# lilinitsy/skele-raytracer

Measured on AMD Instinct MI355X. Metric: Mrays/sec + frame ms, 1920x1080 gillum=16 spheres2.scn, higher is better.
Workload: dtype f32

## Files before the change

skele_raytracer_amd/csrc/launch.h:

```cpp
#pragma once

#include <hip/hip_runtime.h>
#include <stddef.h>
#include <stdint.h>

#include "render_params.h"

enum { SKR_LEVEL0_RUN = 0, SKR_LEVEL0_BUILD, SKR_LEVEL0_REPLAY };
enum { SKR_PIX_NONE = 0, SKR_PIX_NODE, SKR_PIX_BACKGROUND, SKR_PIX_TRIANGLE };

constexpr int SKR_NODE_LEVELS_MAX = 33;
struct NodePlan {
	bool flat = false;
	int levels = 0;
	uint32_t band_nblk = 0;
	uint64_t nodes_max[SKR_NODE_LEVELS_MAX] = {};
	uint32_t cap[SKR_NODE_LEVELS_MAX] = {};
	size_t off_nodes[SKR_NODE_LEVELS_MAX] = {}, off_shade[SKR_NODE_LEVELS_MAX] = {}, off_recs[SKR_NODE_LEVELS_MAX] = {}, off_res[SKR_NODE_LEVELS_MAX] = {}, off_ixh[SKR_NODE_LEVELS_MAX] = {};
	size_t off_ctr = 0, ctr_bytes = 0, total = 0, banded = 0;
	size_t off_cls = 0, off_sums = 0;
	size_t off_girow = 0;
	int level0 = SKR_LEVEL0_RUN;
	size_t lds_leaf = 0;
	size_t lds = 0;
};

constexpr int SKR_GLEVELS_MAX = 64;
struct GPlan {
	int levels = 0;
	uint32_t band_rows = 0;
	uint64_t nodes_max[SKR_GLEVELS_MAX + 1] = {};
	uint32_t cap[SKR_GLEVELS_MAX + 1] = {};
	size_t off_nodes[SKR_GLEVELS_MAX + 1] = {}, off_recs[SKR_GLEVELS_MAX + 1] = {}, off_res[SKR_GLEVELS_MAX + 1] = {}, off_hdr[SKR_GLEVELS_MAX + 1] = {};
	size_t off_ctr = 0, ctr_bytes = 0, total = 0;
};

struct QueryTrees {
	const float4 *tree;
	const float4 *trace;
	uint32_t stride;
	int32_t nchunks;
	int32_t cones, trace_cones;
	float4 ball;
};

struct ShadeRays {
	const float4 *rays;
	const uint32_t *keys;
	float *out;
	uint32_t n, ray0;
	QueryTrees trees;
};
constexpr uint32_t SKR_SHADE_ROW = 1024;

struct TriShadows {
	QueryTrees trees;
};

struct GenericFeatures {
	bool tri_shadows = false;
	bool sphere_tree = false;
	bool spot = false;
	bool soft = false;
	TriShadows shadows{};
	SphereTree stree{};
	SpotLights spots{};
	SoftLights softs{};
};

enum SkrPath { SKR_PATH_DIRECT = 0, SKR_PATH_NODES, SKR_PATH_GENERIC };

struct LaunchPlan {
	SkrPath path = SKR_PATH_DIRECT;
	const char *variant = "direct_v3";
	size_t scratch_bytes = 0;
	size_t acc_bytes = 0;
	size_t lds_bytes = 0;
	size_t off_ctr = 0;
	int levels = 0;
	NodePlan nodes;
	GPlan generic;
	GenericFeatures features;
};

static inline size_t skr_scene_lds_bytes(const RenderParams &p) { return ((size_t) 4 * p.n_spheres + 1 + 2 * p.n_lights) * 16; }

constexpr size_t SKR_PREFIX_LDS = ((size_t) SKR_PREFIX_WORDS * sizeof(uint32_t) + 15) & ~(size_t) 15;
static inline size_t skr_scene_kernels_lds(const RenderParams &p) { return skr_scene_lds_bytes(p) + 32 + SKR_PREFIX_LDS; }
static inline size_t skr_lights_lds_bytes(const RenderParams &p) { return ((size_t) 1 + 2 * p.n_lights) * 16; }
static inline size_t skr_lights_kernels_lds(const RenderParams &p) { return skr_lights_lds_bytes(p) + 32 + SKR_PREFIX_LDS; }

static inline uint32_t skr_tree_arity(const RenderParams &p) { return (uint32_t) (p.monte_carlo ? p.num_path_traces : 0) + (p.legacy_reflect ? 2u * (uint32_t) p.n_lights : 0u); }

struct ScratchLayout {
	size_t off = 0;
	size_t take(size_t bytes) { const size_t o = off; off += (bytes + 255) & ~(size_t) 255; return o; }
};

template <class Fits>
static uint32_t skr_largest_band(uint32_t all, Fits fits)
{
	if(fits(all)) return all;
	uint32_t lo = 1, hi = all;
	if(!fits(lo)) return 0;
	while(hi - lo > 1)
	{
		const uint32_t mid = lo + (hi - lo) / 2;
		if(fits(mid)) lo = mid;
		else hi = mid;
	}
	return lo;
}

enum SkrLeafShape { SKR_LEAF_RUNTIME = 0, SKR_LEAF_POINT1 = 1, SKR_LEAF_POINT2 = 2 };
static inline SkrLeafShape skr_leaf_shape(const RenderParams &p)
{
	if(!(p.sw.shadow_mask & SKR_SW_LEAF_SHAPE)) return SKR_LEAF_RUNTIME;
	if(p.n_tris != 0 || p.gi_index == nullptr || p.gi_wide != 0) return SKR_LEAF_RUNTIME;
	if(!p.use_shadows || p.shadow_masks == nullptr) return SKR_LEAF_RUNTIME;
	if(p.pow_steps > 7) return SKR_LEAF_RUNTIME;
	return p.n_lights == 2 ? SKR_LEAF_POINT2 : p.n_lights == 1 ? SKR_LEAF_POINT1 : SKR_LEAF_RUNTIME;
}

bool skr_plan_launch(const RenderParams &p, size_t lds_limit, LaunchPlan &lp, const GenericFeatures &f);
const char *skr_features_conflict(const GenericFeatures &f, bool legacy_reflect, bool shade_triangles, bool fog);
const char *skr_generic_variant(bool query, const GenericFeatures &f);
hipError_t skr_launch_render(const RenderParams &p, const LaunchPlan &lp, hipStream_t stream, const SkrTimingHook *hook);
hipError_t skr_launch_debug(int op, const void *d_in, void *d_out, uint32_t n, hipStream_t stream);
bool skr_nodes_plan(const RenderParams &p, size_t lds_limit, NodePlan &pl);
hipError_t skr_launch_nodes(const RenderParams &p, const NodePlan &pl, hipStream_t stream, const SkrTimingHook *hook);
hipError_t skr_nodes_level_count(const void *scratch, size_t off_ctr, int level, uint32_t *n);
bool skr_generic_plan(const RenderParams &p, GPlan &pl, bool sphere_tree = false);
hipError_t skr_launch_generic(const RenderParams &p, const GPlan &pl, hipStream_t stream, const SkrTimingHook *hook, const GenericFeatures &f, const ShadeRays *q = nullptr);
struct PrimaryKey {
	int32_t width, height;
	uint32_t tile_rows, first_tile, tile_stride, out_rows;
	const uint32_t *tile_table;
	uint64_t tile_table_id;
	float inv_width, inv_height, aspect, angle;
	f3 cam_pos, cam_dir, cam_up, cam_right, background;
	int32_t n_spheres, n_tris, n_lights;
	const float4 *scene, *cam_ec, *tri_chunks;
	int32_t tri_chunk_size, tri_cones, n_tri_chunks;
	int32_t use_shadows, pow_steps, num_path_traces, max_depth, flat, levels;
	const void *gi_index, *gi_surface;
	uint32_t band_nblk;
	const void *scratch;
	const void *counters;
	size_t off_ctr, off_nodes0, off_shade0, off_cls, off_sums, off_girow, total;
};
bool skr_primary_key(const RenderParams &p, const NodePlan &pl, uint64_t tile_table_id, PrimaryKey &key);
hipError_t skr_launch_wave(const RenderParams &p, size_t lds, hipStream_t stream);
hipError_t skr_launch_primary(const RenderParams &p, dim3 grid, size_t lds, hipStream_t stream);
hipError_t skr_launch_primary_build(const RenderParams &p, dim3 grid, size_t lds, uint8_t *cls, unsigned long long *sums, hipStream_t stream);
hipError_t skr_launch_primary_replay(const RenderParams &p, const uint8_t *cls, const unsigned long long *sums, hipStream_t stream);
hipError_t skr_launch_resolve(const RenderParams &p, hipStream_t stream);
hipError_t skr_launch_camec(const float4 *geom, int ns, f3 cam_pos, float4 *out, hipStream_t stream);
struct TraceScene {
	const float4 *geom;
	const float4 *tris;
	QueryTrees trees;
	int32_t ns, nt, chunk;
	f3 cam;
};
hipError_t skr_launch_trace(const TraceScene &s, const float4 *rays, uint32_t n, bool any_hit, void *out, hipStream_t stream, const SphereTree *st = nullptr);
hipError_t skr_launch_camera_rays(const RenderParams &p, float4 *rays, hipStream_t stream);
struct DenoiseScratch {
	float4 *img[2];
	float4 *guide;
	uint32_t *cls;
};
hipError_t skr_launch_denoise(const DenoiseScratch &b, uint32_t w, uint32_t h, const float *rgbf, const float4 *hits, const float *var, int iterations,
							  float *out_rgbf, uint8_t *out_rgb, hipStream_t stream);
hipError_t skr_launch_accumulate(float *acc, const float *frame, size_t n, int first, hipStream_t stream);
hipError_t skr_launch_resolve_accumulated(const float *acc, uint32_t passes, uint32_t width, uint32_t out_rows, uint32_t height, uint32_t tile_rows,
										  uint32_t first_tile, uint32_t tile_stride, const uint32_t *tile_table, uint8_t *rgb, float *rgbf, hipStream_t stream);
struct AdaptiveScratch {
	float4 *st;
	uint2 *st2;
	uint32_t *list[2];
	uint32_t *blocks;
	uint32_t *count;
	float4 *rays;
	float *shade;
	float *sacc;
};
struct AdaptiveRule {
	uint32_t min_passes, max_passes;
	float threshold;
};
constexpr float SKR_ADAPTIVE_CROSSOVER = 0.5f;
size_t skr_adaptive_scratch_bytes(uint64_t pixels);
AdaptiveScratch skr_adaptive_carve(void *base, uint64_t pixels);
hipError_t skr_launch_adaptive_fold(const AdaptiveScratch &s, const float *frame, const uint32_t *list, uint32_t m, int first, hipStream_t stream);
hipError_t skr_launch_adaptive_select(const AdaptiveScratch &s, const AdaptiveRule &rule, const uint32_t *in, uint32_t m, uint32_t *out, hipStream_t stream);
hipError_t skr_launch_adaptive_rays(const RenderParams &p, const uint32_t *list, uint32_t m, float4 *rays, hipStream_t stream);
hipError_t skr_launch_adaptive_sample(const AdaptiveScratch &s, const uint32_t *list, uint32_t m, uint32_t sample, uint32_t samples, hipStream_t stream);
hipError_t skr_launch_adaptive_resolve(const AdaptiveScratch &s, uint64_t pixels, uint8_t *rgb, float *rgbf, uint32_t *passes, float *var, hipStream_t stream);
```

skele_raytracer_amd/csrc/render_nodes.hip:

```cpp
#include <hip/hip_runtime.h>
#include <stdint.h>
#include <stdlib.h>
#include <string.h>

#include <vector>

#include "launch.h"
#include "wave_common.h"

namespace {

constexpr uint32_t PC_HIT0 = 1u, PC_HIT1 = 2u, PC_BLACK0 = 4u, PC_BLACK1 = 8u;
constexpr int IXH_ROWS = 3;
constexpr int NQ_CAP = 176;
constexpr int NQ_PRE = NQ_CAP - 128;
constexpr int NQ_F = 5;
constexpr int NWIN = 4;
constexpr int WIN_FLOATS = 2 * 3 * 64;
constexpr int LEAF2_WAVE_FLOATS = NQ_CAP * NQ_F + NWIN * WIN_FLOATS;

typedef const RenderParams __attribute__((address_space(4))) *LaunchArgs;
SKR_DEV const RenderParams &launch_args()
{
	LaunchArgs k = (LaunchArgs) __builtin_amdgcn_kernarg_segment_ptr();
	asm volatile("" : "+s"(k));
	return *(const RenderParams *) k;
}

SKR_DEV bool classify_child(const SceneView &sv, f3 co, f3 d, float two_a, float four_a, const BestState &s, bool &black)
{
	black = false;
	if(sv.nt > 0)
	{
		const float tmin = (s.best >= 0) ? near_root(two_a, s.b, s.D) : __builtin_inff();
		black = any_triangle_closer(sv, RayConst{co, d, two_a, four_a}, tmin);
	}
	return !black && s.best >= 0;
}

}

#ifndef SKR_TRACE_LOOP
#define SKR_TRACE_LOOP 1
#endif
#if SKR_TRACE_LOOP
#define SKR_TRACE_STRIDE gridDim.x
#else
#define SKR_TRACE_STRIDE 0x40000000u
#undef SKR_TRACE_GRID_MAX
#define SKR_TRACE_GRID_MAX 0x7fffffffu
#endif
#ifndef SKR_TRACE_WAVES
#define SKR_TRACE_WAVES 0
#endif
#if SKR_TRACE_WAVES
#define SKR_TRACE_ATTR __attribute__((amdgpu_waves_per_eu(SKR_TRACE_WAVES, SKR_TRACE_WAVES)))
#else
#define SKR_TRACE_ATTR
#endif
template <bool TRIS, bool GIM>
__global__ __launch_bounds__(256) SKR_TRACE_ATTR void skr_trace_kernel(const RenderParams)
{
	extern __shared__ __align__(16) unsigned char lds_raw[];
	float4 *lds4 = reinterpret_cast<float4 *>(lds_raw);
	const RenderParams &p = launch_args();
	const uint32_t N = (uint32_t) p.num_path_traces, PP = (N + 1u) >> 1;
	const uint64_t n_pairs = (uint64_t) *p.nd_count * PP;
	if((uint64_t) blockIdx.x * 256u >= n_pairs) return;
	stage_scene(p, lds4, TRIS);
	const int tid = threadIdx.x, lane = tid & 63;
	Counters cn{0, 0, 0};
	for(uint32_t blk = blockIdx.x; (uint64_t) blk * 256u < n_pairs; blk += SKR_TRACE_STRIDE)
	{
	const RenderParams &p = launch_args();
	const SceneView sv = scene_view(p, lds4, TRIS);
	const uint32_t chunk = blk * 4u + (uint32_t) (tid >> 6);
	const uint64_t tp = (uint64_t) chunk * 64u + (uint32_t) lane;
	const bool valid = tp < n_pairs;
	const uint32_t node = valid ? (uint32_t) (tp / PP) : 0u, j = valid ? (uint32_t) (tp - (uint64_t) node * PP) : 0u;
	const bool second = valid && 2u * j + 1u < N;
	bool hit0 = false, hit1 = false;
	float4 rec0 = make_float4(0, 0, 0, 0), rec1 = rec0;
	bool black0 = false, black1 = false;
	if(valid)
	{
		const float4 *row = p.nd_src + (size_t) node * 2;
		const float4 a0 = row[0], a1 = row[1];
		const f3 co = mk3(a0.x, a0.y, a0.z), Nn = mk3(a0.w, a1.x, a1.y);
		const uint32_t pixel = __float_as_uint(a1.z), node_id = __float_as_uint(a1.w);
		f3 nt, nb;
		tangent_basis(Nn, nt, nb);
		uint32_t rnd[4];
		philox4x32(pixel, p.aa_index, node_id, j, p.seed_lo, p.seed_hi, rnd);
		const float q1a = u31_to_unit(rnd[0]), q2a = u31_to_unit(rnd[1]), q1b = u31_to_unit(rnd[2]), q2b = u31_to_unit(rnd[3]);
		const DirPair dp = gi_direction_pair(q1a, q2a, q1b, q2b, Nn, nt, nb);
		const f3 d0 = dp.d0, d1 = dp.d1;
		cn.rays += second ? 2u : 1u;
		const RayPair rp = make_pair(d0, d1);
		BestState s0, s1;
		int gi_row = -1;
		if(GIM) gi_row = p.gi_row0 ? p.gi_row0[node] : gi_origin_row(p, co);
		closest_pair<GIM>(sv, p, gi_row, co, d0, d1, second, rp, s0, s1);
		hit0 = classify_child(sv, co, d0, rp.two_a.x, rp.four_a.x, s0, black0);
		rec0 = make_float4(__uint_as_float(node), __uint_as_float((uint32_t) (s0.best & 0xffff) | ((2u * j) << 16)), q1a, q2a);
		if(second)
		{
			hit1 = classify_child(sv, co, d1, rp.two_a.y, rp.four_a.y, s1, black1);
			rec1 = make_float4(__uint_as_float(node), __uint_as_float((uint32_t) (s1.best & 0xffff) | ((2u * j + 1u) << 16)), q1b, q2b);
		}
	}
	const unsigned long long m0 = __ballot(hit0), m1 = __ballot(hit1);
	const uint32_t region = chunk & (SKR_P1_REGIONS - 1u);
	const uint32_t n0h = (uint32_t) __popcll(m0), n1h = (uint32_t) __popcll(m1);
	uint32_t base = 0;
	if(n0h + n1h != 0u)
	{
		if(lane == 0) base = atomicAdd(lc_count(p.rc_ctr, region), n0h + n1h);
		base = (uint32_t) __builtin_amdgcn_readfirstlane((int) base);
	}
	const uint32_t rec_base = region * p.rc_cap + base;
	const uint32_t rank0 = (uint32_t) lanes_below(m0), rank1 = (uint32_t) lanes_below(m1);
	if(hit0) p.rc[rec_base + rank0] = rec0;
	if(hit1) p.rc[rec_base + n0h + rank1] = rec1;
	if(TRIS)
	{
		const unsigned long long k0 = __ballot(black0), k1 = __ballot(black1);
		if(lane == 0) p.ixh[IXH_ROWS * (size_t) chunk + 2] = make_uint4((uint32_t) k0, (uint32_t) (k0 >> 32), (uint32_t) k1, (uint32_t) (k1 >> 32));
	}
	if(lane == 0)
	{
		p.ixh[IXH_ROWS * (size_t) chunk] = make_uint4(rec_base, n0h, 0u, 0u);
		p.ixh[IXH_ROWS * (size_t) chunk + 1] = make_uint4((uint32_t) m0, (uint32_t) (m0 >> 32), (uint32_t) m1, (uint32_t) (m1 >> 32));
	}
	}
	add_counters(launch_args(), cn, (uint32_t) blockIdx.x * 4u + (uint32_t) (tid >> 6), lane);
}

struct Activated {
	f3 co, N, direct;
	uint32_t pixel, node_id, sph, child;
	float r1;
};

template <typename SH = RunTimeShape>
SKR_DEV Activated activate_record(const SceneView &sv, const RenderParams &p, bool act, uint32_t rec, Counters &cn)
{
	Activated a;
	a.co = a.N = mk3(0, 0, 1);
	a.direct = mk3(0, 0, 0);
	a.pixel = a.node_id = a.sph = a.child = 0;
	a.r1 = 0.0f;
	if(act)
	{
		typedef float v4f __attribute__((ext_vector_type(4)));
		const v4f n0 = __builtin_nontemporal_load(reinterpret_cast<const v4f *>(p.rc + rec));
		const uint32_t parent = __float_as_uint(n0.x), sc = __float_as_uint(n0.y);
		a.r1 = n0.z;
		a.sph = sc & 0xffffu;
		a.child = sc >> 16;
		const float4 *row = p.nd_src + (size_t) parent * 2;
		const float4 p0 = row[0], p1 = row[1];
		const f3 co0 = mk3(p0.x, p0.y, p0.z), N0 = mk3(p0.w, p1.x, p1.y);
		a.pixel = __float_as_uint(p1.z);
		const uint32_t pnode = __float_as_uint(p1.w);
		a.node_id = pnode * (uint32_t) p.num_path_traces + a.child + 1u;
		f3 nt0, nb0;
		tangent_basis(N0, nt0, nb0);
		const f3 d = gi_direction(a.r1, n0.w, N0, nt0, nb0);
		const float4 g = sv.geom[a.sph];
		const f3 ec = co0 - ld3(g);
		const float aa = dot3(d, d);
		const float b = 2 * dot3(d, ec);
		const float D = b * b - (4 * aa) * (dot3(ec, ec) - g.w);
		const float two_a = 2 * aa;
		const float t = near_root(two_a, b, D);
		const f3 P = co0 + d * t;
		a.N = normalize3(P - ld3(sv.geom[a.sph]));
		cn.hits++;
		a.direct = direct_light<false, SH>(sv, p, (int) a.sph, P, a.N, cn);
		a.co = add_scalar(P, 0.00001f);
	}
	return a;
}

#ifndef SKR_SHADE_WAVES
#define SKR_SHADE_WAVES 5
#endif
#if SKR_SHADE_WAVES
#define SKR_SHADE_ATTR __attribute__((amdgpu_waves_per_eu(SKR_SHADE_WAVES, SKR_SHADE_WAVES)))
#else
#define SKR_SHADE_ATTR
#endif
template <bool TRIS>
__global__ __launch_bounds__(256) SKR_SHADE_ATTR void skr_activate_kernel(const RenderParams p)
{
	extern __shared__ __align__(16) unsigned char lds_raw[];
	float4 *lds4 = reinterpret_cast<float4 *>(lds_raw);
	const uint32_t per_region = (p.rc_cap + 255u) / 256u;
	const uint32_t region = (uint32_t) blockIdx.x / per_region, pos0 = ((uint32_t) blockIdx.x % per_region) * 256u;
	const uint32_t cnt = *lc_count(p.rc_ctr, region);
	if(pos0 >= cnt && blockIdx.x != 0) return;
	__shared__ uint32_t s_pre[SKR_PREFIX_WORDS];
	region_prefix(p, s_pre, blockIdx.x == 0);
	if(pos0 >= cnt) return;
	const SceneView sv = stage_scene(p, lds4, TRIS);
	const uint32_t pos = pos0 + threadIdx.x;
	const bool act = pos < cnt;
	const uint32_t rec = region * p.rc_cap + pos;
	Counters cn{0, 0, 0};
	const Activated a = activate_record(sv, p, act, rec, cn);
	if(act)
	{
		const size_t n = (size_t) (s_pre[region] + pos);
		float4 *grow = p.nd_dst + n * 2, *srow = p.ns_dst + n * 2;
		grow[0] = make_float4(a.co.x, a.co.y, a.co.z, a.N.x);
		grow[1] = make_float4(a.N.y, a.N.z, __uint_as_float(a.pixel), __uint_as_float(a.node_id));
		srow[0] = make_float4(a.direct.x, a.direct.y, a.direct.z, __uint_as_float(a.sph));
		srow[1] = make_float4(a.r1, __uint_as_float(rec), __uint_as_float(a.pixel), __uint_as_float(a.node_id));
	}
	add_counters(p, cn, blockIdx.x * 4u + (threadIdx.x >> 6), threadIdx.x & 63);
}

template <bool TRIS>
__global__ __launch_bounds__(256) SKR_SHADE_ATTR void skr_shade_leaf_kernel(const RenderParams p)
{
	extern __shared__ __align__(16) unsigned char lds_raw[];
	float4 *lds4 = reinterpret_cast<float4 *>(lds_raw);
	__shared__ uint32_t prefix[SKR_PREFIX_WORDS];
	region_prefix(p, prefix, false);
	const uint32_t total = prefix[64];
	if((uint32_t) blockIdx.x * 256u >= total) return;
	const SceneView sv = stage_scene(p, lds4, TRIS);
	Counters cn{0, 0, 0};
	for(uint32_t base = (uint32_t) blockIdx.x * 256u; base < total; base += gridDim.x * 256u)
	{
		const uint32_t i = base + threadIdx.x;
		const bool act = i < total;
		uint32_t lo = 0, hi = SKR_P1_REGIONS;
		while(hi - lo > 1u)
		{
			const uint32_t mid = (lo + hi) >> 1;
			if(prefix[mid] <= (act ? i : 0u)) lo = mid;
			else hi = mid;
		}
		const uint32_t rec = lo * p.rc_cap + ((act ? i : 0u) - prefix[lo]);
		const Activated a = activate_record(sv, p, act, rec, cn);
		if(act)
		{
			const f3 tot = mk3(0, 0, 0);
			const f3 colour = (div3_const(a.direct, SKR_DIV_PI) + tot * 2.0f) * ld3(sv.kd[a.sph]);
			store3(p.res_out + (size_t) rec * 3, div3_const(colour * a.r1, SKR_DIV_PDF));
		}
	}
	add_counters(p, cn, blockIdx.x * 4u + (threadIdx.x >> 6), threadIdx.x & 63);
}

namespace {

struct Ring {
	float *base;
	int head, count;
};

SKR_DEV void ring_push(Ring &q, bool pred, f3 d, uint32_t ids, float r1)
{
	const unsigned long long m = __ballot(pred);
	if(pred)
	{
		int e = q.head + q.count + lanes_below(m);
		e -= (e >= NQ_CAP) ? NQ_CAP : 0;
		float *r = q.base + e;
		r[0 * NQ_CAP] = d.x;
		r[1 * NQ_CAP] = d.y;
		r[2 * NQ_CAP] = d.z;
		r[3 * NQ_CAP] = __uint_as_float(ids);
		r[4 * NQ_CAP] = r1;
	}
	q.count = uni(q.count + (int) __popcll(m));
}

template <typename SH>
SKR_DEV void leaf_batch(const SceneView &sv, const RenderParams &p, Ring &q, float *slots, f3 co, int lane, int m, Counters &cn)
{
	wave_lds_fence();
	const bool act = lane < m;
	DIAG_WAVE(9, 1);
	DIAG_WAVE(10, m);
	int e = q.head + (act ? lane : 0);
	e -= (e >= NQ_CAP) ? NQ_CAP : 0;
// ... 179 lines not shown
		const bool act = act0;
		f3 nt, nb;
		tangent_basis(Nn, nt, nb);
		STAMP(1);
		f3 acc = mk3(0, 0, 0);
		for(int jj = 0; jj < R; jj++)
		{
			const int j = jj;
			const bool second = 2 * j + 1 < N;
			float *wrow = slots + (jj & (NWIN - 1)) * WIN_FLOATS + pl;
			if(jj >= NWIN)
			{
				wave_lds_fence();
				for(int c = 0; c < 2; c++) acc = acc + mk3(wrow[(3 * c) * cs], wrow[(3 * c + 1) * cs], wrow[(3 * c + 2) * cs]);
				wave_lds_fence();
			}
			float *win = wrow;
			bool hit0 = false, hit1 = false;
			f3 d0 = mk3(0, 0, 1), d1 = mk3(0, 0, 1);
			float q1a = 0, q1b = 0;
			int s0b = 0, s1b = 0;
			if(act)
			{
				uint32_t rnd[4];
				uint32_t k0 = p.seed_lo, k1 = p.seed_hi;
				asm volatile("" : "+s"(k0), "+s"(k1));
				philox4x32(pixel, p.aa_index, node_id, (uint32_t) j, k0, k1, rnd);
				q1a = u31_to_unit(rnd[0]);
				q1b = u31_to_unit(rnd[2]);
				const float q2a = u31_to_unit(rnd[1]), q2b = u31_to_unit(rnd[3]);
				f3 nq = Nn;
				asm volatile("" : "+v"(nq.x), "+v"(nq.y), "+v"(nq.z));
				const f3 nbr = cross3(nq, nt);
				const DirPair dp = gi_direction_pair(q1a, q2a, q1b, q2b, Nn, nt, nbr);
				d0 = dp.d0;
				d1 = dp.d1;
				cn.rays += second ? 2u : 1u;
				const RayPair rp = make_pair(d0, d1);
				BestState s0, s1;
				closest_pair<GIM, SH>(sv, p, gi_row, co, d0, d1, second, rp, s0, s1);
				bool black;
				hit0 = classify_child(sv, co, d0, rp.two_a.x, rp.four_a.x, s0, black);
				if(!hit0)
				{
					const f3 c = div3_const((black ? mk3(0, 0, 0) : p.background) * q1a, SKR_DIV_PDF);
					win[0] = c.x;
					win[cs] = c.y;
					win[2 * cs] = c.z;
				}
				s0b = s0.best;
				if(second)
				{
					hit1 = classify_child(sv, co, d1, rp.two_a.y, rp.four_a.y, s1, black);
					if(!hit1)
					{
						const f3 c = div3_const((black ? mk3(0, 0, 0) : p.background) * q1b, SKR_DIV_PDF);
						win[3 * cs] = c.x;
						win[4 * cs] = c.y;
						win[5 * cs] = c.z;
					}
					s1b = s1.best;
				}
			}
			STAMP(2);
			const bool last = jj + 1 == R;
			const uint32_t idj = ((uint32_t) lane << 16) | ((uint32_t) jj << 23);
			ring_push(q, hit0, d0, (uint32_t) (s0b & 0xffff) | idj, q1a);
			ring_push(q, hit1, d1, (uint32_t) (s1b & 0xffff) | idj | (1u << 22), q1b);
			for(;;)
			{
				bool go = q.count >= 64 || (!last && q.count > NQ_PRE);
				if(!go && q.count > 0)
				{
					go = last;
					if(!go && jj + 1 >= NWIN)
					{
						wave_lds_fence();
						const uint32_t head_ids = (uint32_t) uni((int) __float_as_uint(q.base[3 * NQ_CAP + q.head]));
						go = (int) (head_ids >> 23) <= jj + 1 - NWIN;
					}
				}
				if(!go) break;
				STAMP(4);
				leaf_batch<SH>(sv, p, q, slots, co, lane, q.count < 64 ? q.count : 64, cn);
				STAMP(3);
			}
			STAMP(4);
		}
		wave_lds_fence();
		for(int jr = (R > NWIN ? R - NWIN : 0); jr < R; jr++)
		{
			const float *wrow = slots + (jr & (NWIN - 1)) * WIN_FLOATS + pl;
			for(int c = 0; c < 2; c++)
				if(2 * jr + c < N) acc = acc + mk3(wrow[(3 * c) * cs], wrow[(3 * c + 1) * cs], wrow[(3 * c + 2) * cs]);
		}
		wave_lds_fence();
		if(act0)
		{
			f3 direct;
			uint32_t sph;
			float r1 = 0.0f;
			if(FIRST)
			{
				direct = direct1;
				sph = __float_as_uint(p.ns_src[(size_t) (first + (uint32_t) lane) * 2].w);
			}
			else
			{
				direct = direct1;
				const float4 r1row = p.rc[out_idx];
				r1 = r1row.z;
				sph = __float_as_uint(r1row.y) & 0xffffu;
			}
			const f3 total = acc / (float) N;
			const f3 colour = (div3_const(direct, SKR_DIV_PI) + total * 2.0f) * ld3(sv.kd[sph]);
			if(FIRST) emit_sample(p, out_idx, colour);
			else store3(p.res_out + (size_t) out_idx * 3, div3_const(colour * r1, SKR_DIV_PDF));
		}
		STAMP(5);
#if defined(SKR_TIMELINE) && SKR_TIMELINE
		wt_units++;
		wt_last = wall_clock64();
#endif
	}
#if defined(SKR_TIMELINE) && SKR_TIMELINE
	if(lane == 0 && g < 4096u)
	{
		skr_leaf2_times[6 * g] = wt_start;
		skr_leaf2_times[6 * g + 1] = wt_first;
		skr_leaf2_times[6 * g + 2] = wt_last;
		skr_leaf2_times[6 * g + 3] = wall_clock64();
		skr_leaf2_times[6 * g + 4] = wt_units;
		skr_leaf2_times[6 * g + 5] = __builtin_readcyclecounter() - wc_start;
	}
#endif
#if defined(SKR_STAMPS) && SKR_STAMPS
	if(p.counters && lane == 0)
		for(int k = 0; k < 8; k++) atomicAdd(&p.counters[4u * SKR_COUNTER_SHARDS + k], st_acc[k]);
#endif
	add_counters(p, cn, g, lane);
}

__global__ __launch_bounds__(256) void skr_finalize_kernel2(const RenderParams p)
{
	const uint32_t n = *p.nd_count;
	const uint32_t node = (uint32_t) blockIdx.x * 256u + threadIdx.x;
	if((uint32_t) blockIdx.x * 256u >= n) return;
	if(node >= n) return;
	const int N = p.num_path_traces, PP = (N + 1) >> 1;
	const float4 *row = p.ns_src + (size_t) node * 2;
	const float4 b0 = row[0], b1 = row[1];
	const uint32_t pixel = __float_as_uint(b1.z), node_id = __float_as_uint(b1.w);
	f3 total = mk3(0, 0, 0);
	for(int j0 = 0; j0 < PP; j0 += 4)
	{
		uint32_t code[4], rec[8];
		f3 v[8];
#pragma unroll
		for(int k = 0; k < 4; k++)
		{
			const uint64_t tp = (uint64_t) node * (uint32_t) PP + (uint32_t) (j0 + k);
			code[k] = 0;
			rec[2 * k] = rec[2 * k + 1] = 0;
			if(j0 + k < PP)
			{
				const uint4 *h = p.ixh + IXH_ROWS * (size_t) (tp >> 6);
				const uint4 h0 = h[0], h1 = h[1];
				const unsigned long long m0 = (unsigned long long) h1.y << 32 | h1.x, m1 = (unsigned long long) h1.w << 32 | h1.z;
				const uint32_t bit = (uint32_t) tp & 63u;
				const unsigned long long below = (1ull << bit) - 1ull;
				code[k] = (uint32_t) ((m0 >> bit) & 1ull) * PC_HIT0 | (uint32_t) ((m1 >> bit) & 1ull) * PC_HIT1;
				if(p.n_tris > 0)
				{
					const uint4 h2 = h[2];
					const unsigned long long k0 = (unsigned long long) h2.y << 32 | h2.x, k1 = (unsigned long long) h2.w << 32 | h2.z;
					code[k] |= (uint32_t) ((k0 >> bit) & 1ull) * PC_BLACK0 | (uint32_t) ((k1 >> bit) & 1ull) * PC_BLACK1;
				}
				rec[2 * k] = h0.x + (uint32_t) __popcll(m0 & below);
				rec[2 * k + 1] = h0.x + h0.y + (uint32_t) __popcll(m1 & below);
			}
		}
#pragma unroll
		for(int k = 0; k < 8; k++)
		{
			v[k] = mk3(0, 0, 0);
			if(code[k >> 1] & ((k & 1) ? PC_HIT1 : PC_HIT0))
			{
				const float *r = p.res_in + (size_t) rec[k] * 3;
				v[k] = mk3(r[0], r[1], r[2]);
			}
		}
#pragma unroll
		for(int k = 0; k < 4; k++)
		{
			if(j0 + k < PP)
			{
				uint32_t rnd[4];
				philox4x32(pixel, p.aa_index, node_id, (uint32_t) (j0 + k), p.seed_lo, p.seed_hi, rnd);
#pragma unroll
				for(int c = 0; c < 2; c++)
				{
					if(2 * (j0 + k) + c < N)
					{
						f3 term = v[2 * k + c];
						if(!(code[k] & (c ? PC_HIT1 : PC_HIT0)))
						{
							const float r1 = u31_to_unit(rnd[2 * c]);
							term = (code[k] & (c ? PC_BLACK1 : PC_BLACK0)) ? mk3(0, 0, 0) : div3_const(p.background * r1, SKR_DIV_PDF);
						}
						total = total + term;
					}
				}
			}
		}
	}
	const f3 direct = mk3(b0.x, b0.y, b0.z);
	const uint32_t sph = __float_as_uint(b0.w);
	total = total / (float) N;
	const f3 colour = (div3_const(direct, SKR_DIV_PI) + total * 2.0f) * ld3(p.sph_kd[sph]);
	if(p.nd_src_level0) emit_sample(p, __float_as_uint(b1.y), colour);
	else store3(p.res_out + (size_t) __float_as_uint(b1.y) * 3, div3_const(colour * b1.x, SKR_DIV_PDF));
}

#ifndef SKR_TRACE_GRID_MAX
#define SKR_TRACE_GRID_MAX 49152u
#endif
#ifndef SKR_FLAT_BELOW
#define SKR_FLAT_BELOW 1.2e7
#endif
static const uint32_t LEAF2_GRID = 256u * SKR_LEAF2_OCC;

static bool nodes_flat_wanted(const RenderParams &p)
{
	if(p.sw.flat) return p.sw.flat > 0;
	double recs = (double) p.width * p.out_rows;
	for(int k = 2; k < p.max_depth; k++) recs *= (double) p.num_path_traces;
	return recs < SKR_FLAT_BELOW;
}

static bool plan_for(const RenderParams &p, uint32_t nblk, bool flat, NodePlan &pl)
{
	const uint64_t N = (uint64_t) p.num_path_traces, PP = (N + 1) >> 1;
	pl.flat = flat;
	pl.levels = p.max_depth - 1 + (flat ? 1 : 0);
	if(pl.levels < 1 || pl.levels > SKR_NODE_LEVELS_MAX) return false;
	pl.band_nblk = nblk;
	pl.nodes_max[0] = (uint64_t) nblk * 256u;
	pl.cap[0] = 0;
	for(int L = 1; L < pl.levels; L++)
	{
		const uint64_t chunks = (pl.nodes_max[L - 1] * PP + 63) / 64;
		const uint64_t cap = (chunks + SKR_P1_REGIONS - 1) / SKR_P1_REGIONS * 128;
		if(cap * SKR_P1_REGIONS >= (1ull << 31)) return false;
		pl.cap[L] = (uint32_t) cap;
		pl.nodes_max[L] = cap * SKR_P1_REGIONS;
	}
	ScratchLayout s;
	pl.ctr_bytes = (SKR_PULL_STRIDE + LVL_CTR_WORDS * (size_t) pl.levels) * sizeof(uint32_t);
	pl.off_ctr = s.take(pl.ctr_bytes);
	for(int L = 0; L < pl.levels; L++)
	{
		const size_t n = (size_t) pl.nodes_max[L];
		if(L > 0)
		{
			pl.off_recs[L] = s.take(n * 16);
			pl.off_res[L] = s.take(n * 12 + 16);
		}
		if(L < pl.levels - 1 || pl.levels == 1)
		{
			pl.off_nodes[L] = s.take(n * 32);
			pl.off_shade[L] = s.take(n * 32);
		}
		if(L < pl.levels - 1)
		{
			pl.off_ixh[L] = s.take(((n * PP + 63) / 64 + 4) * IXH_ROWS * 16);
		}
	}
	pl.banded = s.off - (pl.off_nodes[0]);
	pl.off_cls = s.take((size_t) nblk * 256u);
	pl.off_sums = s.take((size_t) SKR_COUNTER_SHARDS * 4 * sizeof(unsigned long long));
	pl.off_girow = s.take((size_t) nblk * 256u * sizeof(int32_t));
	pl.total = s.off;
	return true;
}

static uint64_t nodes_budget(const RenderParams &p, bool flat)
{
	return p.sw.budget_mb ? (uint64_t) p.sw.budget_mb << 20 : (flat ? 8ull : 4ull) << 30;
}

static bool plan_bands(const RenderParams &p, bool flat, NodePlan &pl)
{
	const uint32_t bx = (uint32_t) (p.width + 15) / 16, by = (p.out_rows + 15) / 16;
	const uint64_t budget = nodes_budget(p, flat);
	uint32_t nblk = skr_largest_band(bx * by, [&](uint32_t n) { return plan_for(p, n, flat, pl) && pl.banded <= budget; });
	if(nblk == 0) return false;
	if(nblk > bx) nblk = nblk / bx * bx;
	return plan_for(p, nblk, flat, pl);
}

bool skr_nodes_plan(const RenderParams &p, size_t lds_limit, NodePlan &pl)
{
	const bool forced = p.sw.pipeline == SKR_PIPE_NODES;
	if(p.sw.pipeline != SKR_PIPE_AUTO && !forced) return false;
	if(p.shade_triangles || p.legacy_reflect) return false;
	if(!(p.monte_carlo && p.n_spheres > 0 && p.n_spheres < 65536 && p.max_depth >= 2 && p.num_path_traces > 0 && p.num_path_traces <= 256)) return false;
	if(!forced && p.n_tris > 64) return false;
	pl.lds_leaf = skr_scene_lds_bytes(p) + 32 + (size_t) 4 * LEAF2_WAVE_FLOATS * sizeof(float);
	if(skr_scene_kernels_lds(p) > lds_limit) return false;
	const bool leaf_fits = pl.lds_leaf <= lds_limit;
	if(nodes_flat_wanted(p) || !leaf_fits)
	{
		const uint32_t all = (uint32_t) ((p.width + 15) / 16) * ((p.out_rows + 15) / 16);
		if(plan_bands(p, true, pl) && (p.sw.flat > 0 || !leaf_fits || pl.band_nblk >= all))
		{
			pl.lds = skr_scene_kernels_lds(p);
			return true;
		}
	}
	pl.lds = pl.lds_leaf;
	return leaf_fits && plan_bands(p, false, pl);
}

hipError_t skr_nodes_level_count(const void *scratch, size_t off_ctr, int level, uint32_t *n)
{
	const uint32_t *ctr = reinterpret_cast<const uint32_t *>(reinterpret_cast<const char *>(scratch) + off_ctr);
	if(level == 0) return hipMemcpy(n, ctr, sizeof(uint32_t), hipMemcpyDeviceToHost);
	std::vector<uint32_t> h((size_t) SKR_P1_REGIONS * SKR_PULL_STRIDE);
	const hipError_t e = hipMemcpy(h.data(), ctr + SKR_PULL_STRIDE + LVL_CTR_WORDS * (size_t) level, h.size() * sizeof(uint32_t), hipMemcpyDeviceToHost);
	if(e != hipSuccess) return e;
	uint64_t total = 0;
	for(uint32_t k = 0; k < SKR_P1_REGIONS; k++) total += h[(size_t) SKR_PULL_STRIDE * k];
	*n = (uint32_t) total;
	return hipSuccess;
}

typedef void (*LeafKernel)(const RenderParams);
template <bool FIRST>
static LeafKernel leaf_instance(const RenderParams &p)
{
	switch(skr_leaf_shape(p))
	{
	case SKR_LEAF_POINT2: return skr_leaf_kernel2<false, FIRST, true, PointLightShape<2>>;
	case SKR_LEAF_POINT1: return skr_leaf_kernel2<false, FIRST, true, PointLightShape<1>>;
	default: break;
	}
	if(p.n_tris > 0) return skr_leaf_kernel2<true, FIRST, false>;
	return p.gi_index != nullptr ? skr_leaf_kernel2<false, FIRST, true> : skr_leaf_kernel2<false, FIRST, false>;
}

template <bool FIRST>
static hipError_t launch_leaf2(const RenderParams &p, size_t lds, hipStream_t stream)
{
	const LeafKernel fn = leaf_instance<FIRST>(p);
	hipError_t e = hipFuncSetAttribute(reinterpret_cast<const void *>(fn), hipFuncAttributeMaxDynamicSharedMemorySize, (int) lds);
	if(e != hipSuccess) return e;
	hipLaunchKernelGGL(fn, dim3(LEAF2_GRID), dim3(256), lds, stream, p);
	return hipGetLastError();
}

hipError_t skr_launch_nodes(const RenderParams &p_in, const NodePlan &pl, hipStream_t stream, const SkrTimingHook *hook)
{
	RenderParams p = p_in;
	char *base = reinterpret_cast<char *>(p.node_scratch);
	uint32_t *ctr0 = reinterpret_cast<uint32_t *>(base + pl.off_ctr);
	auto lvl_ctr = [&](int L) { return ctr0 + SKR_PULL_STRIDE + LVL_CTR_WORDS * (size_t) L; };
	auto nodes = [&](int L) { return reinterpret_cast<float4 *>(base + pl.off_nodes[L]); };
	auto shade = [&](int L) { return reinterpret_cast<float4 *>(base + pl.off_shade[L]); };
	const int nsamp = p.grid_size > 0 ? p.grid_size * p.grid_size : 1;
	const size_t lds_scene = skr_scene_lds_bytes(p) + 32;
	const bool tris = p.n_tris > 0;
	const bool flat = pl.flat;
	const int D = p.max_depth, last = flat ? D - 1 : D - 2;
	const uint32_t blocks_x = (uint32_t) (p.width + 15) / 16, blocks = blocks_x * ((p.out_rows + 15) / 16);
	p.blocks_x = blocks_x;
	p.qctr = ctr0;
	hipError_t e = hipSuccess;
	for(int s = 0; s < nsamp; s++)
	{
		p.aa_index = (uint32_t) s;
		for(uint32_t blk0 = 0; blk0 < blocks; blk0 += pl.band_nblk)
		{
			const bool timed = hook && s == nsamp - 1 && blk0 == 0;
			p.band_blk0 = blk0;
			p.band_nblk = blocks - blk0 < pl.band_nblk ? blocks - blk0 : pl.band_nblk;
			p.nd_dst = nodes(0);
			p.ns_dst = shade(0);
			uint8_t *cls = reinterpret_cast<uint8_t *>(base + pl.off_cls);
			unsigned long long *sums = reinterpret_cast<unsigned long long *>(base + pl.off_sums);
			int32_t *const gi_row0 = pl.level0 != SKR_LEVEL0_RUN ? reinterpret_cast<int32_t *>(base + pl.off_girow) : nullptr;
			p.gi_row0 = gi_row0;
			if(pl.level0 == SKR_LEVEL0_REPLAY)
			{
				e = hipMemsetAsync(ctr0 + SKR_PULL_STRIDE, 0, pl.ctr_bytes - SKR_PULL_STRIDE * sizeof(uint32_t), stream);
				if(e == hipSuccess) e = skr_launch_primary_replay(p, cls, sums, stream);
			}
			else
			{
				e = hipMemsetAsync(ctr0, 0, pl.ctr_bytes, stream);
				if(e == hipSuccess)
					e = pl.level0 == SKR_LEVEL0_BUILD ? skr_launch_primary_build(p, dim3(p.band_nblk), lds_scene, cls, sums, stream)
													  : skr_launch_primary(p, dim3(p.band_nblk), lds_scene, stream);
			}
			if(e != hipSuccess) return e;
			if(D == 2 && !flat)
			{
				p.nd_src = nodes(0);
				p.ns_src = shade(0);
				p.nd_src_level0 = 1;
				p.nd_count = ctr0;
				p.rc_ctr = lvl_ctr(0);
				if(timed) skr_hook_start(hook, stream);
				e = launch_leaf2<true>(p, pl.lds_leaf, stream);
				if(timed) skr_hook_stop(hook, stream);
				if(e != hipSuccess) return e;
				continue;
			}
			for(int L = 1; L <= last; L++)
			{
				p.nd_src = nodes(L - 1);
				p.ns_src = shade(L - 1);
				p.nd_src_level0 = L == 1;
				p.gi_row0 = L == 1 ? gi_row0 : nullptr;
				p.nd_count = L == 1 ? ctr0 : lc_prefix_host(lvl_ctr(L - 1));
				p.rc = reinterpret_cast<float4 *>(base + pl.off_recs[L]);
				p.rc_cap = pl.cap[L];
				p.rc_ctr = lvl_ctr(L);
				p.ixh = reinterpret_cast<uint4 *>(base + pl.off_ixh[L - 1]);
				const uint64_t wg_t = (pl.nodes_max[L - 1] * (uint64_t) ((p.num_path_traces + 1) >> 1) + 255) / 256;
				const unsigned grid_t = (unsigned) (wg_t < SKR_TRACE_GRID_MAX ? wg_t : SKR_TRACE_GRID_MAX);
				if(flat && L == last && timed) skr_hook_start(hook, stream);
				if(tris) hipLaunchKernelGGL((skr_trace_kernel<true, false>), dim3(grid_t), dim3(256), lds_scene, stream, p);
				else if(p.gi_index) hipLaunchKernelGGL((skr_trace_kernel<false, true>), dim3(grid_t), dim3(256), lds_scene, stream, p);
				else hipLaunchKernelGGL((skr_trace_kernel<false, false>), dim3(grid_t), dim3(256), lds_scene, stream, p);
				if(L < last)
				{
					p.nd_dst = nodes(L);
					p.ns_dst = shade(L);
					const unsigned grid_a = SKR_P1_REGIONS * ((pl.cap[L] + 255u) / 256u);
					if(tris) hipLaunchKernelGGL(skr_activate_kernel<true>, dim3(grid_a), dim3(256), lds_scene, stream, p);
					else hipLaunchKernelGGL(skr_activate_kernel<false>, dim3(grid_a), dim3(256), lds_scene, stream, p);
				}
			}
			p.res_out = reinterpret_cast<float *>(base + pl.off_res[last]);
			if(flat)
			{
				const uint64_t wg = (pl.nodes_max[last] + 255) / 256;
				const unsigned grid_s = (unsigned) (wg < 16384 ? wg : 16384);
				if(tris) hipLaunchKernelGGL(skr_shade_leaf_kernel<true>, dim3(grid_s), dim3(256), lds_scene, stream, p);
				else hipLaunchKernelGGL(skr_shade_leaf_kernel<false>, dim3(grid_s), dim3(256), lds_scene, stream, p);
				if(timed) skr_hook_stop(hook, stream);
			}
			else
			{
				if(timed) skr_hook_start(hook, stream);
				e = launch_leaf2<false>(p, pl.lds_leaf, stream);
				if(timed) skr_hook_stop(hook, stream);
				if(e != hipSuccess) return e;
			}
			for(int L = last - 1; L >= 0; L--)
			{
				p.nd_src = nodes(L);
				p.ns_src = shade(L);
				p.nd_src_level0 = L == 0;
				p.nd_count = L == 0 ? ctr0 : lc_prefix_host(lvl_ctr(L));
				p.ixh = reinterpret_cast<uint4 *>(base + pl.off_ixh[L]);
				p.res_in = reinterpret_cast<const float *>(base + pl.off_res[L + 1]);
				p.res_out = L == 0 ? nullptr : reinterpret_cast<float *>(base + pl.off_res[L]);
				hipLaunchKernelGGL(skr_finalize_kernel2, dim3((unsigned) ((pl.nodes_max[L] + 255) / 256)), dim3(256), 0, stream, p);
			}
			e = hipGetLastError();
			if(e != hipSuccess) return e;
		}
	}
	if(p.grid_size > 0) return skr_launch_resolve(p, stream);
	return hipSuccess;
}
```

Before: 69900.

## Trace GI rays node-major so each wave reuses node data across sample pairs

The GI trace kernel now gives each wave 64 consecutive nodes and a run of sample-pair indices, where before it spread flattened (node, pair) indices across lanes. Lanes in a wave share the same pair index and the tangent basis and GI row are computed once per node run. Header rows are now indexed by node block times pair count, and the resolve/activate lookups and scratch sizing are updated to match. This is meant to improve coherence and cut repeated node loads, but a wave wastes lanes when a node block is only partly filled and more header rows may be allocated.

```diff
diff --git a/skele_raytracer_amd/csrc/launch.h b/skele_raytracer_amd/csrc/launch.h
--- a/skele_raytracer_amd/csrc/launch.h
+++ b/skele_raytracer_amd/csrc/launch.h
@@ -111,6 +111,24 @@
 	}
 	return lo;
 }
+
+#ifndef SKR_TRACE_BY_NODE
+#define SKR_TRACE_BY_NODE 1
+#endif
+#ifndef SKR_TRACE_RUN
+#define SKR_TRACE_RUN 2
+#endif
+__host__ __device__ static inline uint64_t skr_trace_header_row(uint64_t node, uint32_t j, uint32_t PP)
+{
+	return SKR_TRACE_BY_NODE ? (node >> 6) * PP + j : (node * PP + j) >> 6;
+}
+__host__ __device__ static inline uint32_t skr_trace_header_bit(uint64_t node, uint32_t j, uint32_t PP)
+{
+	return (uint32_t) (SKR_TRACE_BY_NODE ? node : node * PP + j) & 63u;
+}
+static inline uint64_t skr_trace_rows_used(uint64_t nodes, uint64_t PP) { return SKR_TRACE_BY_NODE ? (nodes + 63) / 64 * PP : (nodes * PP + 63) / 64; }
+static inline uint64_t skr_trace_rows_alloc(uint64_t nodes, uint64_t PP) { return skr_trace_rows_used(nodes, PP) + 4; }
+static inline uint64_t skr_trace_region_cap(uint64_t nodes, uint64_t PP) { return (skr_trace_rows_used(nodes, PP) + SKR_P1_REGIONS - 1) / SKR_P1_REGIONS * 128; }
 
 enum SkrLeafShape { SKR_LEAF_RUNTIME = 0, SKR_LEAF_POINT1 = 1, SKR_LEAF_POINT2 = 2 };
 static inline SkrLeafShape skr_leaf_shape(const RenderParams &p)
diff --git a/skele_raytracer_amd/csrc/render_nodes.hip b/skele_raytracer_amd/csrc/render_nodes.hip
--- a/skele_raytracer_amd/csrc/render_nodes.hip
+++ b/skele_raytracer_amd/csrc/render_nodes.hip
@@ -58,6 +58,125 @@
 #else
 #define SKR_TRACE_ATTR
 #endif
+template <bool TRIS, bool GIM>
+SKR_DEV void trace_round(const SceneView &sv, const RenderParams &p, bool valid, uint32_t node, uint32_t j, f3 co, f3 Nn, f3 nt, f3 nb, uint32_t pixel,
+						 uint32_t node_id, int gi_row, uint32_t chunk, int lane, Counters &cn)
+{
+	const uint32_t N = (uint32_t) p.num_path_traces;
+	const bool second = valid && 2u * j + 1u < N;
+	bool hit0 = false, hit1 = false;
+	float4 rec0 = make_float4(0, 0, 0, 0), rec1 = rec0;
+	bool black0 = false, black1 = false;
+	if(valid)
+	{
+		uint32_t rnd[4];
+		philox4x32(pixel, p.aa_index, node_id, j, p.seed_lo, p.seed_hi, rnd);
+		const float q1a = u31_to_unit(rnd[0]), q2a = u31_to_unit(rnd[1]), q1b = u31_to_unit(rnd[2]), q2b = u31_to_unit(rnd[3]);
+		const DirPair dp = gi_direction_pair(q1a, q2a, q1b, q2b, Nn, nt, nb);
+		const f3 d0 = dp.d0, d1 = dp.d1;
+		cn.rays += second ? 2u : 1u;
+		const RayPair rp = make_pair(d0, d1);
+		BestState s0, s1;
+		closest_pair<GIM>(sv, p, gi_row, co, d0, d1, second, rp, s0, s1);
+		hit0 = classify_child(sv, co, d0, rp.two_a.x, rp.four_a.x, s0, black0);
+		rec0 = make_float4(__uint_as_float(node), __uint_as_float((uint32_t) (s0.best & 0xffff) | ((2u * j) << 16)), q1a, q2a);
+		if(second)
+		{
+			hit1 = classify_child(sv, co, d1, rp.two_a.y, rp.four_a.y, s1, black1);
+			rec1 = make_float4(__uint_as_float(node), __uint_as_float((uint32_t) (s1.best & 0xffff) | ((2u * j + 1u) << 16)), q1b, q2b);
+		}
+	}
+	const unsigned long long m0 = __ballot(hit0), m1 = __ballot(hit1);
+	const uint32_t region = chunk & (SKR_P1_REGIONS - 1u);
+	const uint32_t n0h = (uint32_t) __popcll(m0), n1h = (uint32_t) __popcll(m1);
+	uint32_t base = 0;
+	if(n0h + n1h != 0u)
+	{
+		if(lane == 0) base = atomicAdd(lc_count(p.rc_ctr, region), n0h + n1h);
+		base = (uint32_t) __builtin_amdgcn_readfirstlane((int) base);
+	}
+	const uint32_t rec_base = region * p.rc_cap + base;
+	const uint32_t rank0 = (uint32_t) lanes_below(m0), rank1 = (uint32_t) lanes_below(m1);
+	if(hit0) p.rc[rec_base + rank0] = rec0;
+	if(hit1) p.rc[rec_base + n0h + rank1] = rec1;
+	if(TRIS)
+	{
+		const unsigned long long k0 = __ballot(black0), k1 = __ballot(black1);
+		if(lane == 0) p.ixh[IXH_ROWS * (size_t) chunk + 2] = make_uint4((uint32_t) k0, (uint32_t) (k0 >> 32), (uint32_t) k1, (uint32_t) (k1 >> 32));
+	}
+	if(lane == 0)
+	{
+		p.ixh[IXH_ROWS * (size_t) chunk] = make_uint4(rec_base, n0h, 0u, 0u);
+		p.ixh[IXH_ROWS * (size_t) chunk + 1] = make_uint4((uint32_t) m0, (uint32_t) (m0 >> 32), (uint32_t) m1, (uint32_t) (m1 >> 32));
+	}
+}
+
+__host__ __device__ static inline uint32_t trace_run(uint32_t PP) { return SKR_TRACE_RUN > 0 && (uint32_t) SKR_TRACE_RUN < PP ? (uint32_t) SKR_TRACE_RUN : PP; }
+__host__ __device__ static inline uint32_t trace_runs_per_block(uint32_t PP) { return (PP + trace_run(PP) - 1u) / trace_run(PP); }
+
+#if SKR_TRACE_BY_NODE
+template <bool TRIS, bool GIM>
+__global__ __launch_bounds__(256) SKR_TRACE_ATTR void skr_trace_kernel(const RenderParams)
+{
+	extern __shared__ __align__(16) unsigned char lds_raw[];
+	float4 *lds4 = reinterpret_cast<float4 *>(lds_raw);
+	const RenderParams &p = launch_args();
+	const uint32_t PP0 = ((uint32_t) p.num_path_traces + 1u) >> 1;
+	const uint32_t items = ((*p.nd_count + 63u) >> 6) * trace_runs_per_block(PP0);
+	if((uint64_t) blockIdx.x * 4u >= items) return;
+	stage_scene(p, lds4, TRIS);
+	const int tid = threadIdx.x, lane = tid & 63;
+	const uint32_t wave = (uint32_t) uni(tid >> 6);
+	Counters cn{0, 0, 0};
+	for(uint32_t blk = blockIdx.x; (uint64_t) blk * 4u < items; blk += SKR_TRACE_STRIDE)
+	{
+		const uint32_t item = blk * 4u + wave;
+		if(item >= items) break;
+		uint32_t j0, j1, node;
+		bool valid;
+		f3 nt = mk3(0, 1, 0);
+		int gi_row = -1;
+		{
+			const RenderParams &p = launch_args();
+			const uint32_t PP = ((uint32_t) p.num_path_traces + 1u) >> 1, RPB = trace_runs_per_block(PP), RUN = trace_run(PP);
+			const uint32_t B = item / RPB;
+			j0 = (item - B * RPB) * RUN;
+			j1 = j0 + RUN < PP ? j0 + RUN : PP;
+			node = B * 64u + (uint32_t) lane;
+			valid = node < *p.nd_count;
+			if(valid)
+			{
+				const float4 *row = p.nd_src + (size_t) node * 2;
+				const float4 a0 = row[0], a1 = row[1];
+				const f3 co = mk3(a0.x, a0.y, a0.z), Nn = mk3(a0.w, a1.x, a1.y);
+				f3 nb;
+				tangent_basis(Nn, nt, nb);
+				if(GIM) gi_row = p.gi_row0 ? p.gi_row0[node] : gi_origin_row(p, co);
+			}
+		}
+		for(uint32_t j = j0; j < j1; j++)
+		{
+			const RenderParams &p = launch_args();
+			const SceneView sv = scene_view(p, lds4, TRIS);
+			f3 co = mk3(0, 0, 1), Nn = mk3(0, 0, 1);
+			uint32_t pixel = 0, node_id = 0;
+			if(valid)
+			{
+				const float4 *row = p.nd_src + (size_t) node * 2;
+				const float4 a0 = row[0], a1 = row[1];
+				co = mk3(a0.x, a0.y, a0.z);
+				Nn = mk3(a0.w, a1.x, a1.y);
+				pixel = __float_as_uint(a1.z);
+				node_id = __float_as_uint(a1.w);
+			}
+			const f3 nb = cross3(Nn, nt);
+			const uint32_t chunk = (node >> 6) * (((uint32_t) p.num_path_traces + 1u) >> 1) + j;
+			trace_round<TRIS, GIM>(sv, p, valid, node, j, co, Nn, nt, nb, pixel, node_id, gi_row, (uint32_t) uni((int) chunk), lane, cn);
+		}
+	}
+	add_counters(launch_args(), cn, (uint32_t) blockIdx.x * 4u + wave, lane);
+}
+#else
 template <bool TRIS, bool GIM>
 __global__ __launch_bounds__(256) SKR_TRACE_ATTR void skr_trace_kernel(const RenderParams)
 {
@@ -78,63 +197,25 @@
 	const uint64_t tp = (uint64_t) chunk * 64u + (uint32_t) lane;
 	const bool valid = tp < n_pairs;
 	const uint32_t node = valid ? (uint32_t) (tp / PP) : 0u, j = valid ? (uint32_t) (tp - (uint64_t) node * PP) : 0u;
-	const bool second = valid && 2u * j + 1u < N;
-	bool hit0 = false, hit1 = false;
-	float4 rec0 = make_float4(0, 0, 0, 0), rec1 = rec0;
-	bool black0 = false, black1 = false;
+	f3 co = mk3(0, 0, 1), Nn = mk3(0, 0, 1), nt = mk3(0, 1, 0), nb = mk3(1, 0, 0);
+	uint32_t pixel = 0, node_id = 0;
+	int gi_row = -1;
 	if(valid)
 	{
 		const float4 *row = p.nd_src + (size_t) node * 2;
 		const float4 a0 = row[0], a1 = row[1];
-		const f3 co = mk3(a0.x, a0.y, a0.z), Nn = mk3(a0.w, a1.x, a1.y);
-		const uint32_t pixel = __float_as_uint(a1.z), node_id = __float_as_uint(a1.w);
-		f3 nt, nb;
+		co = mk3(a0.x, a0.y, a0.z);
+		Nn = mk3(a0.w, a1.x, a1.y);
+		pixel = __float_as_uint(a1.z);
+		node_id = __float_as_uint(a1.w);
 		tangent_basis(Nn, nt, nb);
-		uint32_t rnd[4];
-		philox4x32(pixel, p.aa_index, node_id, j, p.seed_lo, p.seed_hi, rnd);
-		const float q1a = u31_to_unit(rnd[0]), q2a = u31_to_unit(rnd[1]), q1b = u31_to_unit(rnd[2]), q2b = u31_to_unit(rnd[3]);
-		const DirPair dp = gi_direction_pair(q1a, q2a, q1b, q2b, Nn, nt, nb);
-		const f3 d0 = dp.d0, d1 = dp.d1;
-		cn.rays += second ? 2u : 1u;
-		const RayPair rp = make_pair(d0, d1);
-		BestState s0, s1;
-		int gi_row = -1;
 		if(GIM) gi_row = p.gi_row0 ? p.gi_row0[node] : gi_origin_row(p, co);
-		closest_pair<GIM>(sv, p, gi_row, co, d0, d1, second, rp, s0, s1);
-		hit0 = classify_child(sv, co, d0, rp.two_a.x, rp.four_a.x, s0, black0);
-		rec0 = make_float4(__uint_as_float(node), __uint_as_float((uint32_t) (s0.best & 0xffff) | ((2u * j) << 16)), q1a, q2a);
-		if(second)
-		{
-			hit1 = classify_child(sv, co, d1, rp.two_a.y, rp.four_a.y, s1, black1);
-			rec1 = make_float4(__uint_as_float(node), __uint_as_float((uint32_t) (s1.best & 0xffff) | ((2u * j + 1u) << 16)), q1b, q2b);
-		}
-	}
-	const unsigned long long m0 = __ballot(hit0), m1 = __ballot(hit1);
-	const uint32_t region = chunk & (SKR_P1_REGIONS - 1u);
-	const uint32_t n0h = (uint32_t) __popcll(m0), n1h = (uint32_t) __popcll(m1);
-	uint32_t base = 0;
-	if(n0h + n1h != 0u)
-	{
-		if(lane == 0) base = atomicAdd(lc_count(p.rc_ctr, region), n0h + n1h);
-		base = (uint32_t) __builtin_amdgcn_readfirstlane((int) base);
-	}
-	const uint32_t rec_base = region * p.rc_cap + base;
-	const uint32_t rank0 = (uint32_t) lanes_below(m0), rank1 = (uint32_t) lanes_below(m1);
-	if(hit0) p.rc[rec_base + rank0] = rec0;
-	if(hit1) p.rc[rec_base + n0h + rank1] = rec1;
-	if(TRIS)
-	{
-		const unsigned long long k0 = __ballot(black0), k1 = __ballot(black1);
-		if(lane == 0) p.ixh[IXH_ROWS * (size_t) chunk + 2] = make_uint4((uint32_t) k0, (uint32_t) (k0 >> 32), (uint32_t) k1, (uint32_t) (k1 >> 32));
-	}
-	if(lane == 0)
-	{
-		p.ixh[IXH_ROWS * (size_t) chunk] = make_uint4(rec_base, n0h, 0u, 0u);
-		p.ixh[IXH_ROWS * (size_t) chunk + 1] = make_uint4((uint32_t) m0, (uint32_t) (m0 >> 32), (uint32_t) m1, (uint32_t) (m1 >> 32));
-	}
+	}
+	trace_round<TRIS, GIM>(sv, p, valid, node, j, co, Nn, nt, nb, pixel, node_id, gi_row, chunk, lane, cn);
 	}
 	add_counters(launch_args(), cn, (uint32_t) blockIdx.x * 4u + (uint32_t) (tid >> 6), lane);
 }
+#endif
 
 struct Activated {
 	f3 co, N, direct;
@@ -620,6 +701,9 @@
 	const float4 b0 = row[0], b1 = row[1];
 	const uint32_t pixel = __float_as_uint(b1.z), node_id = __float_as_uint(b1.w);
 	f3 total = mk3(0, 0, 0);
+#if SKR_TRACE_BY_NODE
+	const uint32_t hrow0 = (uint32_t) uni((int) (node >> 6)) * (uint32_t) PP;
+#endif
 	for(int j0 = 0; j0 < PP; j0 += 4)
 	{
 		uint32_t code[4], rec[8];
@@ -627,15 +711,21 @@
 #pragma unroll
 		for(int k = 0; k < 4; k++)
 		{
+#if SKR_TRACE_BY_NODE
+			const size_t hrow = (size_t) hrow0 + (uint32_t) (j0 + k);
+			const uint32_t bit = node & 63u;
+#else
 			const uint64_t tp = (uint64_t) node * (uint32_t) PP + (uint32_t) (j0 + k);
+			const size_t hrow = (size_t) (tp >> 6);
+			const uint32_t bit = (uint32_t) tp & 63u;
+#endif
 			code[k] = 0;
 			rec[2 * k] = rec[2 * k + 1] = 0;
 			if(j0 + k < PP)
 			{
-				const uint4 *h = p.ixh + IXH_ROWS * (size_t) (tp >> 6);
+				const uint4 *h = p.ixh + IXH_ROWS * hrow;
 				const uint4 h0 = h[0], h1 = h[1];
 				const unsigned long long m0 = (unsigned long long) h1.y << 32 | h1.x, m1 = (unsigned long long) h1.w << 32 | h1.z;
-				const uint32_t bit = (uint32_t) tp & 63u;
 				const unsigned long long below = (1ull << bit) - 1ull;
 				code[k] = (uint32_t) ((m0 >> bit) & 1ull) * PC_HIT0 | (uint32_t) ((m1 >> bit) & 1ull) * PC_HIT1;
 				if(p.n_tris > 0)
@@ -717,8 +807,7 @@
 	pl.cap[0] = 0;
 	for(int L = 1; L < pl.levels; L++)
 	{
-		const uint64_t chunks = (pl.nodes_max[L - 1] * PP + 63) / 64;
-		const uint64_t cap = (chunks + SKR_P1_REGIONS - 1) / SKR_P1_REGIONS * 128;
+		const uint64_t cap = skr_trace_region_cap(pl.nodes_max[L - 1], PP);
 		if(cap * SKR_P1_REGIONS >= (1ull << 31)) return false;
 		pl.cap[L] = (uint32_t) cap;
 		pl.nodes_max[L] = cap * SKR_P1_REGIONS;
@@ -741,7 +830,7 @@
 		}
 		if(L < pl.levels - 1)
 		{
-			pl.off_ixh[L] = s.take(((n * PP + 63) / 64 + 4) * IXH_ROWS * 16);
+			pl.off_ixh[L] = s.take((size_t) skr_trace_rows_alloc(n, PP) * IXH_ROWS * 16);
 		}
 	}
 	pl.banded = s.off - (pl.off_nodes[0]);
@@ -750,6 +839,24 @@
 	pl.off_girow = s.take((size_t) nblk * 256u * sizeof(int32_t));
 	pl.total = s.off;
 	return true;
+}
+
+extern "C" uint32_t skr_trace_header_map(uint32_t nodes, uint32_t N, uint64_t *out, uint32_t *rows, uint32_t *bits)
+{
+	const uint32_t PP = (N + 1u) >> 1;
+	if(out)
+	{
+		out[0] = skr_trace_rows_used(nodes, PP);
+		out[1] = skr_trace_rows_alloc(nodes, PP);
+		out[2] = skr_trace_region_cap(nodes, PP);
+	}
+	for(uint32_t n = 0; n < nodes && rows && bits; n++)
+		for(uint32_t j = 0; j < PP; j++)
+		{
+			rows[(size_t) n * PP + j] = (uint32_t) skr_trace_header_row(n, j, PP);
+			bits[(size_t) n * PP + j] = skr_trace_header_bit(n, j, PP);
+		}
+	return PP;
 }
 
 static uint64_t nodes_budget(const RenderParams &p, bool flat)
@@ -895,7 +1002,11 @@
 				p.rc_cap = pl.cap[L];
 				p.rc_ctr = lvl_ctr(L);
 				p.ixh = reinterpret_cast<uint4 *>(base + pl.off_ixh[L - 1]);
+#if SKR_TRACE_BY_NODE
+				const uint64_t wg_t = ((pl.nodes_max[L - 1] + 63) / 64 * trace_runs_per_block(((uint32_t) p.num_path_traces + 1u) >> 1) + 3) / 4;
+#else
 				const uint64_t wg_t = (pl.nodes_max[L - 1] * (uint64_t) ((p.num_path_traces + 1) >> 1) + 255) / 256;
+#endif
 				const unsigned grid_t = (unsigned) (wg_t < SKR_TRACE_GRID_MAX ? wg_t : SKR_TRACE_GRID_MAX);
 				if(flat && L == last && timed) skr_hook_start(hook, stream);
 				if(tris) hipLaunchKernelGGL((skr_trace_kernel<true, false>), dim3(grid_t), dim3(256), lds_scene, stream, p);
```

Result: faster. 70710 (median of 6 runs) (+1.2%).
